# binbinmeng/QCNN_GPU

Hardware: NVIDIA B200
Metric: luma Mpixel/s (QVRCNN int8, 1080p) (higher is better)
Workload: dtype int8

## Files before the change

### include/qvrcnn_b200.h

```cpp
#ifndef QVRCNN_B200_H
#define QVRCNN_B200_H

#include <stddef.h>
#include <stdint.h>

#ifdef __cplusplus
extern "C" {
#endif

#if defined(__GNUC__)
#define QV_API __attribute__((visibility("default")))
#else
#define QV_API
#endif

typedef struct qv_net qv_net;

enum {
    QV_OK = 0,
    QV_ERR_ARG = -1,
    QV_ERR_IO = -2,
    QV_ERR_CUDA = -3,
    QV_ERR_RANGE = -4,
    QV_ERR_STATE = -5
// ... 15 lines not shown
QV_API int qv_destroy(qv_net *net);

QV_API int qv_load_static_para(qv_net *net, const char *filename);
QV_API int qv_load_static_para_mem(qv_net *net, const void *image, size_t len);
QV_API int qv_load_static_para_hwcn(qv_net *net, const char *filename);

QV_API int qv_load_quant_params(qv_net *net, const char *filename);
QV_API int qv_read_quant_params(const char *filename, int32_t *out18);
QV_API int qv_set_weights(qv_net *net, int layer, const int8_t *w_kcrs, const int32_t *bias);
QV_API int qv_get_quant_params(const qv_net *net, int32_t *out18);

QV_API int qv_load_data(qv_net *net, const uint8_t *host_luma);
QV_API int qv_forward_blu(qv_net *net);
QV_API int qv_get_recon(qv_net *net, uint8_t *host_out);

QV_API int qv_forward_frames_host(qv_net *net, const uint8_t *h_in, uint8_t *h_out, int n_frames);
QV_API int qv_stream_yuv(qv_net *net, const char *anchor_yuv, const char *ori_yuv, const char *recon_yuv,
                         int first_frame, int n_frames, int64_t *sse_before, int64_t *sse_after);
QV_API int qv_stream_yuv_pf(qv_net *net, const char *anchor_yuv, const char *ori_yuv, const char *recon_yuv,
                            int first_frame, int n_frames, int64_t *sse_before_pf, int64_t *sse_after_pf);
QV_API int qv_forward_frames_device(qv_net *net, const uint8_t *d_in, uint8_t *d_out, int n_frames,
                                    void *cuda_stream);
QV_API int qv_forward_frames_device_sse(qv_net *net, const uint8_t *d_in, const uint8_t *d_ori, uint8_t *d_out,
                                        int n_frames, int64_t *d_sse, void *cuda_stream);
QV_API int qv_forward_rows_device(qv_net *net, const uint8_t *d_in, int img_height, int in_row0, int in_rows,
                                  uint8_t *d_out, int out_row0, int out_row1, void *cuda_stream);

QV_API int qv_synchronize(qv_net *net, void *cuda_stream);

typedef struct { unsigned char opaque[192]; } qv_strip_desc;
enum { QV_STRIP_ABOVE = 0, QV_STRIP_BELOW = 1 };
QV_API int qv_strip_setup(qv_net *net, int img_height, int row0, int row1);
QV_API int qv_strip_export(qv_net *net, qv_strip_desc *out);
QV_API int qv_strip_attach(qv_net *net, int side, const qv_strip_desc *neighbour);
QV_API int qv_strip_input(qv_net *net, int slot, void **d_rows);
QV_API int qv_strip_acquire(qv_net *net, int slot, void *cuda_stream);
QV_API int qv_strip_load(qv_net *net, int slot, const uint8_t *host_rows, void *cuda_stream);
QV_API int qv_strip_forward(qv_net *net, int slot, uint8_t *d_out, void *cuda_stream);
QV_API int qv_strip_forward_sse(qv_net *net, int slot, const uint8_t *d_ori_rows, uint8_t *d_out, int64_t *d_sse2,
                                void *cuda_stream);
QV_API int qv_strip_release(qv_net *net);

QV_API int qv_device_buffers(qv_net *net, void **d_x, void **d_x_rec);

QV_API int qv_sse_device(const uint8_t *d_a, const uint8_t *d_b, size_t n, int64_t *d_sse_accum, void *cuda_stream);

QV_API int qv_set_impl(qv_net *net, int impl);
QV_API int qv_get_impl(const qv_net *net);
QV_API long long qv_launch_count(const qv_net *net);
QV_API int qv_get_activation(qv_net *net, int which , int8_t *host_out);

QV_API int qv_debug_fused_tables(const void *model_image, size_t len, uint8_t *wimg, uint32_t *ops, int32_t *consts, size_t sizes[3]);

QV_API int qv_debug_fused_units(int sm_count, int n_frames, int height, int width, int row0, int row1, int row_window, int allow_line,
                                int32_t *units, size_t *n_units, int *grid);

QV_API int qv_convert_model_hwcn_to_vect_c(const char *file_in, const char *file_out);

QV_API int qv_solve_quant_params(const double *stepw_in, const double *blu_in, double *rows_out36);
QV_API int qv_write_quant_params_cpp(const char *filename, const double *rows36);
QV_API int qv_quantize_layer(const float *w, size_t n_w, const float *b, size_t n_b, double stepw, double ratio,
                             int8_t *w_q, int32_t *b_q);

QV_API void *qv_host_alloc(size_t bytes);
QV_API void qv_host_free(void *p);

QV_API int qv_yuv_read_luma(const char *filename, int frames, int height, int width, uint8_t *out);
QV_API int qv_yuv_read_frame(const char *filename, int n, int height, int width, uint8_t *out);
QV_API int qv_yuv_write_recon(const char *filename, const uint8_t *luma, int frames, int height, int width);
QV_API double qv_psnr(const uint8_t *data, const uint8_t *ori, size_t n, int64_t *sse_out);
QV_API double qv_psnr_from_sse(int64_t sse, size_t n);

#ifdef __cplusplus
}
#endif
#endif
```

### qcnn_gpu_b200/api.py

```python
from __future__ import annotations

import ctypes as C
import os
from typing import Optional

import numpy as np

_PKG = os.path.dirname(os.path.abspath(__file__))
LIB_PATH = os.environ.get("QVRCNN_B200_LIB", os.path.join(_PKG, "libqvrcnn_b200.so"))

IMPL_AUTO, IMPL_LAYERED, IMPL_FUSED = 0, 1, 2

ABI_SYMBOLS = (
    "qv_last_error", "qv_version", "qv_create", "qv_destroy", "qv_load_static_para",
    "qv_load_static_para_mem", "qv_load_static_para_hwcn", "qv_load_quant_params", "qv_read_quant_params",
    "qv_set_weights", "qv_get_quant_params", "qv_load_data", "qv_forward_blu", "qv_get_recon",
    "qv_forward_frames_host", "qv_stream_yuv", "qv_stream_yuv_pf", "qv_forward_frames_device", "qv_forward_frames_device_sse", "qv_forward_rows_device", "qv_device_buffers",
    "qv_sse_device", "qv_host_alloc", "qv_host_free",
    "qv_set_impl", "qv_get_impl", "qv_launch_count", "qv_get_activation",
    "qv_convert_model_hwcn_to_vect_c", "qv_yuv_read_luma", "qv_yuv_read_frame", "qv_yuv_write_recon",
    "qv_psnr", "qv_psnr_from_sse", "qv_solve_quant_params", "qv_write_quant_params_cpp", "qv_quantize_layer",
    "qv_debug_fused_tables", "qv_debug_fused_units", "qv_synchronize",
    "qv_strip_setup", "qv_strip_export", "qv_strip_attach", "qv_strip_input", "qv_strip_acquire", "qv_strip_load",
    "qv_strip_forward", "qv_strip_forward_sse", "qv_strip_release",
)

CUDA_STREAM_LEGACY = 1
STRIP_ABOVE, STRIP_BELOW = 0, 1
STRIP_DESC_BYTES = 192


def stream_arg(stream: int):
    return CUDA_STREAM_LEGACY if not stream else stream


class QVError(RuntimeError):
    def __init__(self, code: int, msg: str):
        super().__init__("qvrcnn_b200 error %d: %s" % (code, msg))
        self.code = code


_lib = None


def lib():
    global _lib
    if _lib is None:
        if not os.path.exists(LIB_PATH):
            raise ImportError("%s not found: build it with `python -c 'import __graft_entry__ as g; g.build()'` "
                              "(there is no fallback implementation)" % LIB_PATH)
        L = C.CDLL(LIB_PATH)
        vp, i32, cp = C.c_void_p, C.c_int, C.c_char_p
        L.qv_last_error.restype = cp
        L.qv_version.restype = cp
        L.qv_create.argtypes = [i32, i32, i32, i32, i32, C.POINTER(vp)]
        L.qv_destroy.argtypes = [vp]
        L.qv_load_static_para.argtypes = [vp, cp]
        L.qv_load_static_para_mem.argtypes = [vp, vp, C.c_size_t]
        L.qv_load_static_para_hwcn.argtypes = [vp, cp]
        L.qv_load_quant_params.argtypes = [vp, cp]
        L.qv_read_quant_params.argtypes = [cp, vp]
        L.qv_set_weights.argtypes = [vp, i32, vp, vp]
        L.qv_get_quant_params.argtypes = [vp, vp]
        L.qv_load_data.argtypes = [vp, vp]
        L.qv_forward_blu.argtypes = [vp]
        L.qv_get_recon.argtypes = [vp, vp]
        L.qv_forward_frames_host.argtypes = [vp, vp, vp, i32]
        L.qv_forward_frames_device.argtypes = [vp, vp, vp, i32, vp]
        L.qv_forward_frames_device_sse.argtypes = [vp, vp, vp, vp, i32, vp, vp]
        L.qv_host_alloc.argtypes = [C.c_size_t]
        L.qv_host_alloc.restype = vp
        L.qv_host_free.argtypes = [vp]
        L.qv_host_free.restype = None
        L.qv_stream_yuv.argtypes = [vp, cp, cp, cp, i32, i32, C.POINTER(C.c_int64), C.POINTER(C.c_int64)]
        L.qv_stream_yuv_pf.argtypes = [vp, cp, cp, cp, i32, i32, vp, vp]
# ... 257 lines not shown
```

### qcnn_gpu_b200/csrc/qv_api.cu

```cuda
#include <algorithm>
#include <atomic>
#include <condition_variable>
#include <cstdio>
#include <cstdlib>
#include <cstring>
#include <mutex>
#include <random>
#include <thread>
#include <vector>

#include <fcntl.h>
#include <unistd.h>

#include <cuda_runtime.h>

#include "qv_fused.h"
#include "qv_internal.h"
#include "qv_layered.h"

using namespace qv;

#define QV_CUDA(expr)                                                                       \
    do {                                                                                    \
        cudaError_t e__ = (expr);                                                           \
// ... 243 lines not shown
    *out = net;
    return QV_OK;
}

int qv_destroy(qv_net *net)
{
    if (!net) return QV_OK;
    cudaSetDevice(net->dev);
    if (net->st) cudaStreamSynchronize(net->st);
    qv_strip_release(net);
    free_layered(net);
    if (net->fm) fused_free(net->fm);
    cudaFree(net->d_x); cudaFree(net->d_rec);
    cudaFree(net->d_a1); cudaFree(net->d_a2); cudaFree(net->d_a3);
    cudaFree(net->d_rows_tmp);
    for (int i = 0; i < 2; ++i) {
        cudaFree(net->d_slot_in[i]); cudaFree(net->d_slot_out[i]);
        cudaFreeHost(net->h_pin_in[i]); cudaFreeHost(net->h_pin_out[i]);
        if (net->pst[i]) cudaStreamDestroy(net->pst[i]);
    }
    if (net->ev_compute) cudaEventDestroy(net->ev_compute);
    if (net->st) cudaStreamDestroy(net->st);
    delete net;
    return QV_OK;
}

int qv_load_static_para_mem(qv_net *net, const void *image, size_t len)
{
    if (!net || !image) { set_error("qv_load_static_para_mem: null argument"); return QV_ERR_ARG; }
    ModelHost m;
    int rc = parse_model_vect_c((const uint8_t *)image, len, m);
    if (rc) return rc;
    net->model = m;
    return sync_model(net);
}

int qv_debug_fused_tables(const void *image, size_t len, uint8_t *wimg, uint32_t *ops, int32_t *consts, size_t sizes[3])
{
    if (!image || !sizes) { set_error("qv_debug_fused_tables: null argument"); return QV_ERR_ARG; }
    ModelHost m;
    int rc = parse_model_vect_c((const uint8_t *)image, len, m);
    if (rc) return rc;
    std::vector<uint8_t> w;
    std::vector<uint32_t> o;
    std::vector<int32_t> c;
    fused_debug_tables(m, w, o, c);
    if (wimg && sizes[0] >= w.size()) memcpy(wimg, w.data(), w.size());
    if (ops && sizes[1] >= o.size()) memcpy(ops, o.data(), o.size() * sizeof(uint32_t));
    if (consts && sizes[2] >= c.size()) memcpy(consts, c.data(), c.size() * sizeof(int32_t));
    sizes[0] = w.size(); sizes[1] = o.size(); sizes[2] = c.size();
    return QV_OK;
}

int qv_debug_fused_units(int sm_count, int n_frames, int height, int width, int row0, int row1, int row_window, int allow_line,
                         int32_t *units, size_t *n_units, int *grid)
{
    if (!n_units || !grid) { set_error("qv_debug_fused_units: null argument"); return QV_ERR_ARG; }
    std::vector<int> u;
    int g = 0;
    if (fused_debug_units(sm_count, n_frames, height, width, row0, row1, row_window != 0, allow_line != 0, u, g)) {
        set_error("qv_debug_fused_units: bad geometry");
        return QV_ERR_ARG;
    }
    if (units && *n_units >= u.size() / 5) memcpy(units, u.data(), u.size() * sizeof(int));
    *n_units = u.size() / 5;
    *grid = g;
    return QV_OK;
}

int qv_load_static_para(qv_net *net, const char *filename)
{
    if (!net) { set_error("qv_load_static_para: null handle"); return QV_ERR_ARG; }
    std::vector<uint8_t> buf;
    int rc = read_file(filename, buf);
    if (rc) { set_error("cannot open model file. (%s)", filename ? filename : "(null)"); return rc; }
    return qv_load_static_para_mem(net, buf.data(), buf.size());
}

int qv_load_static_para_hwcn(qv_net *net, const char *filename)
{
    if (!net) { set_error("qv_load_static_para_hwcn: null handle"); return QV_ERR_ARG; }
    std::vector<uint8_t> buf;
    int rc = read_file(filename, buf);
    if (rc) return rc;
    ModelHost m;
    rc = parse_model_hwcn(buf.data(), buf.size(), m);
    if (rc) return rc;
    net->model = m;
    return sync_model(net);
}

int qv_load_quant_params(qv_net *net, const char *filename)
{
    if (!net) { set_error("qv_load_quant_params: null handle"); return QV_ERR_ARG; }
    int32_t q[18];
    int rc = qv_read_quant_params(filename, q);
    if (rc) return rc;
    for (int l = 0; l < QV_NLAYER; ++l) {
        LayerHost &L = net->model.L[l];
        L.blu = q[3 * l]; L.mul = q[3 * l + 1]; L.shift = q[3 * l + 2];
        L.have_q = true;
    }
    return sync_model(net);
}

int qv_set_weights(qv_net *net, int layer, const int8_t *w_kcrs, const int32_t *bias)
// ... 719 lines not shown
```

### qcnn_gpu_b200/csrc/qv_fused.cu

```cuda
#include <algorithm>
#include <cstdio>
#include <cstdlib>
#include <cstring>
#include <mutex>
#include <type_traits>
#include <vector>

#include <cuda.h>
#include <cuda_runtime.h>

#include "qv_device.cuh"
#include "qv_fused.h"
#include "qv_tcgen05.cuh"


#ifndef QV_EXP
#define QV_EXP 0
#endif
#ifndef QV_CODE_SHIFT
#define QV_CODE_SHIFT 5
#endif
#ifndef QV_SHIFT_WORK
#define QV_SHIFT_WORK 0
#endif
#ifndef QV_SHIFT_C4
#define QV_SHIFT_C4 0
#endif
#ifndef QV_BULK_WEIGHTS
#define QV_BULK_WEIGHTS 1
#endif
#ifndef QV_LIGHT_PROF
#define QV_LIGHT_PROF 0
#endif

namespace qv {
namespace {
using namespace tc;
constexpr int EXP = QV_EXP;

constexpr int WT = 120;
constexpr int PW = 136;
constexpr int PLANE = PW * 16;
constexpr int A_SLOTS = 3, IN_SLOTS = 32, IN_PITCH = 144;
constexpr int A1_ROW = 4 * PLANE, A2_ROW = 3 * PLANE;
constexpr int IM_BYTES = 2 * 128 * 16;
constexpr int ZERO_BYTES = 2 * 128 * 16;

constexpr int NR22 = 11 * 16, NR21 = 7 * 32, NR31 = 7 * 16, NR32 = 32;
constexpr int W1_BYTES = 2 * 64 * 16;
constexpr int T22 = 2 * NR22 * 16, T21 = 2 * NR21 * 16, T31 = 2 * NR31 * 16, T32 = 2 * NR32 * 16;
constexpr int OFF_W1 = 0;
constexpr int OFF_W22 = OFF_W1 + W1_BYTES;
constexpr int OFF_W21 = OFF_W22 + 10 * T22;
constexpr int OFF_W31 = OFF_W21 + 6 * T21;
constexpr int OFF_W32 = OFF_W31 + 5 * T31;
constexpr int OFF_BIAS = OFF_W32 + 2 * T32;
constexpr int BIAS_INTS = 64 + 48 + 48;
constexpr int WIMG_BYTES = OFF_BIAS + BIAS_INTS * 4;
constexpr int OFF_A1 = (WIMG_BYTES + 127) / 128 * 128;
constexpr int OFF_A2 = OFF_A1 + A_SLOTS * A1_ROW;
constexpr int OFF_IM = OFF_A2 + A_SLOTS * A2_ROW;
constexpr int OFF_ZERO = OFF_IM + 3 * IM_BYTES;
constexpr int OFF_IN = OFF_ZERO + ZERO_BYTES;
constexpr int OFF_A3 = (OFF_IN + IN_SLOTS * IN_PITCH + 15) / 16 * 16;
constexpr int OFF_CTRL = OFF_A3 + A_SLOTS * A2_ROW;
constexpr int SMEM_BYTES = OFF_CTRL + 64;
static_assert(SMEM_BYTES <= 232448, "exceeds the 227 KB of dynamic shared memory per CTA");
constexpr int IN_PITCH_T = 256, IN_BOX = 144;
constexpr int OFF_IN_T = (SMEM_BYTES + 127) / 128 * 128;
constexpr int SMEM_BYTES_T = OFF_IN_T + IN_SLOTS * IN_PITCH_T;
static_assert(SMEM_BYTES_T <= 232448, "exceeds the 227 KB of dynamic shared memory per CTA");

#ifndef QV_ONE_WORKER
#define QV_ONE_WORKER 1
#endif
constexpr int NWORKER = QV_ONE_WORKER ? 128 : 256, NC4 = 128, NTHREADS = NWORKER + 32 + NC4;
constexpr int MMA_WARP = NWORKER / 32;
constexpr int TR_ITER0 = 300, TR_N = 8;
constexpr int PIPE = 14;

constexpr int TM_D1 = 0;
constexpr int TM_R22 = 128;
constexpr int TM_R21 = 224;
constexpr int TM_R31 = 352;
constexpr int TM_D32 = 416;
constexpr int TM_COLS = 512;

struct GroupQ {
    int hi;
    unsigned M;
    int blu, mul, shift, rbias;
};

struct alignas(64) FusedParams {
    CUtensorMap tmap_in;
    const uint8_t *in;
    uint8_t *out;
    const uint8_t *wimg;
    int n_frames, H, W, nstrips, nseg, seg_rows, n_units, linear, perm_q, perm_s0, perm_r;
    int ys, ye, own0, own1, rlo, rhi;
    size_t frame_stride;
    const uint8_t *in_top, *in_bot;
    const uint32_t *flag_top, *flag_bot;
    uint32_t *pub, *done, *done_ctr;
    uint32_t seq;
    GroupQ q1, q22, q21, q31, q32;
    int c4_bias, c4_mul, c4_shift;
    int c4_w[108];
    long long *dbg;
    uint32_t sbase16, tmem_base;
    int *fail_flag;
    int dbg_flags;
    int bias[BIAS_INTS];
    const uint8_t *ori;
    unsigned long long *sse;
};

struct PhaseBases {
    uint32_t im, a1_r2, a2_r6, b22;
    uint32_t b21, b31, d1, d32;
    uint32_t z22, z21, z31, pad;
};
struct FixedBases { uint32_t zeroA, w1, w32, r22, r21, r31, pad0, pad1; };
constexpr int N_PHASE = 12;
constexpr int N_MMA = 27;
struct PhaseOps {
    uint4 ab[N_MMA];
    uint32_t d1, d32, z22, z21, z31, pad[3];
};
__constant__ PhaseOps c_ops[N_PHASE];

__host__ __device__ __forceinline__ int mod_pos(int a, int m) { int r = a % m; return r < 0 ? r + m : r; }

__host__ __device__ __forceinline__ int wrap_sub(int c, int k, int n) { const int v = c - (k % n); return v < 0 ? v + n : v; }
__host__ __device__ __forceinline__ int wrap_inc(int c, int n) { return c + 1 == n ? 0 : c + 1; }

__device__ __forceinline__ void warp_wait(uint64_t *bar, uint32_t parity, int lane, int *fail)
{
    if (lane == 0 && !tc::mbar_wait(bar, parity)) *fail = 1;
    __syncwarp();
}

__device__ __forceinline__ bool peer_wait(const uint32_t *flag, uint32_t seq)
{
    for (int n = 0; n < 4000000; ++n) {
        uint32_t v;
        asm volatile("ld.acquire.sys.global.u32 %0, [%1];" : "=r"(v) : "l"(flag) : "memory");
        if ((int)(v - seq) >= 0) return true;
        __nanosleep(200);
    }
    return false;
}

struct UnitGeo { int strip, f, y0, y1; bool ok; };
template <bool ROWS>
__host__ __device__ __forceinline__ UnitGeo unit_geo(const FusedParams &P, int unit, int H, int grid)
{
    UnitGeo g;
    if (!ROWS && P.linear) {
        const int b = unit % grid, j = unit / grid;
        const int lo = b * P.seg_rows, hi = min(P.n_frames * P.nstrips * H, lo + P.seg_rows), c = lo / H + j;
        const int start = j == 0 ? lo : c * H, end = min(hi, (c + 1) * H);
        const int full = P.perm_r * (P.perm_s0 + 1);
        const int q = c < full ? c / (P.perm_s0 + 1) : P.perm_r + (c - full) / P.perm_s0;
        const int sl = c < full ? c - q * (P.perm_s0 + 1) : (c - full) - (q - P.perm_r) * P.perm_s0;
        const int col = q + sl * P.perm_q;
        g.f = col / P.nstrips;
        g.strip = col - g.f * P.nstrips;
        g.y0 = start - c * H;
        g.y1 = g.y0 + (end - start);
        g.ok = start < end;
    } else if (!ROWS) {
        const int seg = unit % P.nseg;
        g.strip = (unit / P.nseg) % P.nstrips;
        g.f = unit / (P.nseg * P.nstrips);
        g.y0 = seg * P.seg_rows;
        g.y1 = min(H, g.y0 + P.seg_rows);
        g.ok = true;
    } else {
        const int R = P.ye - P.ys, b = unit % grid, j = unit / grid;
        const int lo = b * P.seg_rows, hi = min(P.nstrips * R, lo + P.seg_rows), c0 = lo / R;
        const int start = j == 0 ? lo : (c0 + j) * R, end = min(hi, (c0 + j + 1) * R);
        g.strip = c0 + j;
// ... 48 lines not shown
    for (int dy = 0; dy < 3; ++dy)
#pragma unroll
        for (int pl = 0; pl < 3; ++pl) {
            const int *w = &P.c4_w[((dy * 3 + DX) * 3 + pl) * 4];
            acc[dy] = __dp4a((int)v[pl].x, w[0], acc[dy]);
            acc[dy] = __dp4a((int)v[pl].y, w[1], acc[dy]);
            acc[dy] = __dp4a((int)v[pl].z, w[2], acc[dy]);
            acc[dy] = __dp4a((int)v[pl].w, w[3], acc[dy]);
        }
}

template <bool FAST, bool PROF, bool ROWS, bool TMA = false>
__global__ void __launch_bounds__(NTHREADS, 1) k_fused(const __grid_constant__ FusedParams P)
{
    constexpr bool SSE = false;
#include "qv_fused_body.inc"
}

template <bool FAST, bool ROWS>
__global__ void __launch_bounds__(NTHREADS, 1) k_enh_sse(const __grid_constant__ FusedParams P)
{
    constexpr bool SSE = true, PROF = false, TMA = false;
#include "qv_fused_body.inc"
}

__global__ void k_wait_words(const uint32_t *a, uint32_t va, const uint32_t *b, uint32_t vb, int *fail_flag)
{
    const uint32_t *w = threadIdx.x == 0 ? a : b;
    const uint32_t v = threadIdx.x == 0 ? va : vb;
    if (w && !peer_wait(w, v)) { *reinterpret_cast<volatile int *>(fail_flag) = 3; __threadfence_system(); }
}

__global__ void k_bases(uint32_t *out)
{
    extern __shared__ __align__(1024) uint8_t sm[];
    uint32_t *slot = reinterpret_cast<uint32_t *>(sm);
    tmem_alloc(slot, TM_COLS);
    tmem_relinquish();
    fence_before_sync();
    __syncwarp();
    fence_after_sync();
    const uint32_t tm = *slot;
    if (threadIdx.x == 0) { out[0] = smem_u32(sm); out[1] = tm; }
    __syncwarp();
    tmem_dealloc(tm, TM_COLS);
}

void build_mma_bases(uint32_t sb, uint32_t tm, PhaseBases *pb, FixedBases &fb)
{
    constexpr uint32_t LP = (uint32_t)(PLANE >> 4) << 16;
    const uint32_t w22 = sb + (OFF_W22 >> 4) + ((uint32_t)NR22 << 16), w21 = sb + (OFF_W21 >> 4) + ((uint32_t)NR21 << 16);
    const uint32_t w31 = sb + (OFF_W31 >> 4) + ((uint32_t)NR31 << 16);
    fb = FixedBases{};
    fb.zeroA = sb + (OFF_ZERO >> 4) + ((128u * 16 >> 4) << 16);
    fb.w1 = sb + (OFF_W1 >> 4) + (64u << 16);
    fb.w32 = sb + (OFF_W32 >> 4) + ((uint32_t)NR32 << 16);
    fb.r22 = tm + TM_R22; fb.r21 = tm + TM_R21; fb.r31 = tm + TM_R31;
    for (int ph = 0; ph < N_PHASE; ++ph) {
        const int R1p = ph + 4096 / N_PHASE * N_PHASE + N_PHASE, c3 = ph % 3, c6 = ph % 6;
        const uint32_t par = ph & 1;
        const int qa = wrap_sub(c6, 2, 6);
        PhaseBases &e = pb[ph];
        e = PhaseBases{};
        e.im = sb + ((OFF_IM + c3 * IM_BYTES) >> 4) + ((128u * 16 >> 4) << 16);
        e.a1_r2 = sb + (OFF_A1 >> 4) + wrap_sub(c3, 2, 3) * (A1_ROW >> 4) + LP;
        e.a2_r6 = sb + (OFF_A2 >> 4) + c3 * (A2_ROW >> 4);
        e.b22 = w22 + (qa <= 2 ? 2 - qa : 8 - qa) * 16;
        e.b21 = w21 + ((1 - (R1p - 2)) & 3) * 32;
        e.b31 = w31 + ((1 - (R1p - 6)) & 3) * 16;
        e.d1 = tm + TM_D1 + par * 64; e.d32 = tm + TM_D32 + par * 32;
        e.z22 = tm + TM_R22 + c6 * 16;
        e.z21 = tm + TM_R21 + ((R1p - 1) & 3) * 32;
        e.z31 = tm + TM_R31 + ((R1p - 5) & 3) * 16;
    }
}

void build_mma_ops(const PhaseBases *pb, const FixedBases &fb, PhaseOps *ops)
{
    constexpr uint32_t HI = (128u >> 4) | (1u << 14);
    constexpr uint32_t LP = (uint32_t)(PLANE >> 4) << 16, LX = 1u << 16;
    for (int ph = 0; ph < N_PHASE; ++ph) {
        const PhaseBases &e = pb[ph];
        PhaseOps &o = ops[ph];
        o = PhaseOps{};
        int k = 0;
        auto put = [&](uint32_t a, uint32_t b) { o.ab[k++] = make_uint4(a, HI, b, HI); };
        put(e.im, fb.w1);
        put(fb.zeroA, fb.w1); put(fb.zeroA, fb.w1); put(fb.zeroA, fb.w1);
        put(e.a2_r6 + 6 + LP, e.b31);
        put(e.a2_r6 + 7 + LP, e.b31 + (T31 >> 4));
        put(e.a2_r6 + 7 + LP, fb.w32);
        put(e.a2_r6 + 8 + LP, e.b31 + 2 * (T31 >> 4));
        put(e.a2_r6 + ((2 * PLANE) >> 4) + 6 + LX, e.b31 + 3 * (T31 >> 4));
        put(e.a2_r6 + ((2 * PLANE) >> 4) + 6 + LX, fb.w32 + (T32 >> 4));
        put(e.a2_r6 + ((2 * PLANE) >> 4) + 8 + LX, e.b31 + 4 * (T31 >> 4));
        for (int t = 0; t < 10; ++t) {
            const int sft = t / 2, h = t & 1;
            const uint32_t a = e.a1_r2 + ((h * 2 * PLANE + (4 + sft) * 16) >> 4);
            put(a, e.b22 + t * (T22 >> 4));
            if (sft >= 1 && sft <= 3) put(a, e.b21 + ((sft - 1) * 2 + h) * (T21 >> 4));
        }
        o.d1 = e.d1; o.d32 = e.d32; o.z22 = e.z22; o.z21 = e.z21; o.z31 = e.z31;
    }
}

}

struct FusedModel {
    int *h_fail = nullptr;
    uint8_t *d_wimg = nullptr;
    FusedParams proto{};
    bool fast = true;
    int sm_count = 148;
    bool env_profile = false, env_test_fail = false, env_tma = false, env_linear = true;
    int env_experiment = 0;
    void *encode_tiled = nullptr;
};

static std::mutex g_ops_mu;
struct OpsRecord { bool done = false; uint32_t sbase16 = 0, tmem_base = 0; };
static OpsRecord g_ops_done[64];

static void put_chunk(uint8_t *blk, int NR, int j, int n, const int8_t *src16) { memcpy(blk + ((size_t)j * NR + n) * 16, src16, 16); }

static bool build_host_image(const ModelHost &m, std::vector<uint8_t> &img, FusedParams &P)
{
    img.assign(WIMG_BYTES, 0);
    auto Wt = [&](int l, int k, int c, int r, int s) -> int8_t {
        const LayerShape &sh = kLayers[l];
        return m.L[l].w[(((size_t)k * sh.cin + c) * sh.k + r) * sh.k + s];
    };
    for (int n = 0; n < 64; ++n) {
        int8_t k32[32] = {0};
        for (int r = 0; r < 5; ++r) {
            for (int s = 0; s < 4; ++s) k32[4 * r + s] = Wt(QV_C1, n, 0, r, s);
            k32[20 + r] = Wt(QV_C1, n, 0, r, 4);
        }
        put_chunk(img.data() + OFF_W1, 64, 0, n, k32);
        put_chunk(img.data() + OFF_W1, 64, 1, n, k32 + 16);
    }
    const int S22[11] = {4, 3, 2, 1, 0, -1, 4, 3, 2, 1, 0};
    const int S3[7] = {2, 1, 0, -1, 2, 1, 0};
    int8_t c16[16];
    for (int s = 0; s < 5; ++s)
        for (int h = 0; h < 2; ++h) {
            uint8_t *blk = img.data() + OFF_W22 + (s * 2 + h) * T22;
            for (int bi = 0; bi < 11; ++bi)
                if (S22[bi] >= 0)
                    for (int j = 0; j < 2; ++j)
                        for (int ch = 0; ch < 16; ++ch) {
                            for (int b = 0; b < 16; ++b) c16[b] = Wt(QV_C2_2, ch, 32 * h + 16 * j + b, S22[bi], s);
                            put_chunk(blk, NR22, j, bi * 16 + ch, c16);
                        }
        }
// ... 27 lines not shown
                }
    for (int ch = 0; ch < 32; ++ch)
        for (int pl = 0; pl < 3; ++pl) {
            for (int b = 0; b < 16; ++b) c16[b] = Wt(QV_C3_2, ch, 16 * pl + b, 0, 0);
            put_chunk(img.data() + OFF_W32 + (pl / 2) * T32, NR32, pl == 2 ? 1 : pl, ch, c16);
        }
    auto mkq = [&](int l, GroupQ &g) -> bool {
        const LayerHost &L = m.L[l];
        g.blu = L.blu; g.mul = L.mul; g.shift = L.shift; g.rbias = (1 << (L.shift - 1)) / L.mul;
        g.hi = L.blu + g.rbias;
        const long long top = ((long long)L.blu + g.rbias) * L.mul;
        const bool ok = L.shift <= 24 && L.mul < (1ll << L.shift) && top < (1ll << 31) && (top >> L.shift) == 127 && g.hi < (1 << 30);
        g.M = ok ? (unsigned)((unsigned long long)L.mul << (24 - L.shift)) : 0u;
        return ok;
    };
    bool fast = true;
    fast &= mkq(QV_C1, P.q1); fast &= mkq(QV_C2_2, P.q22); fast &= mkq(QV_C2_1, P.q21);
    fast &= mkq(QV_C3_1, P.q31); fast &= mkq(QV_C3_2, P.q32);
    int *bias = reinterpret_cast<int *>(img.data() + OFF_BIAS);
    auto addb = [&](int l, int dst0, const GroupQ &g) {
        for (int k = 0; k < kLayers[l].cout; ++k) bias[dst0 + k] = m.L[l].b[k] + (fast ? g.rbias : 0);
    };
    addb(QV_C1, 0, P.q1);
    addb(QV_C2_2, 64, P.q22); addb(QV_C2_1, 64 + 16, P.q21);
    addb(QV_C3_1, 112, P.q31); addb(QV_C3_2, 112 + 16, P.q32);
    memcpy(P.bias, bias, sizeof(P.bias));
    P.c4_bias = m.L[QV_C4].b[0]; P.c4_mul = m.L[QV_C4].mul; P.c4_shift = m.L[QV_C4].shift;
    for (int t = 0; t < 9; ++t)
        for (int pl = 0; pl < 3; ++pl)
            for (int j = 0; j < 4; ++j) {
                unsigned v = 0;
                for (int b = 0; b < 4; ++b) v |= (unsigned)(uint8_t)Wt(QV_C4, 0, 16 * pl + 4 * j + b, t / 3, t % 3) << (8 * b);
                P.c4_w[(t * 3 + pl) * 4 + j] = (int)v;
            }
    return fast;
}

void fused_debug_tables(const ModelHost &m, std::vector<uint8_t> &wimg, std::vector<uint32_t> &ops, std::vector<int32_t> &consts)
{
    FusedParams P{};
    const bool fast = build_host_image(m, wimg, P);
    PhaseBases pb[N_PHASE];
    FixedBases fb;
    build_mma_bases(0, 0, pb, fb);
    std::vector<PhaseOps> po(N_PHASE);
    build_mma_ops(pb, fb, po.data());
    ops.assign(reinterpret_cast<const uint32_t *>(po.data()), reinterpret_cast<const uint32_t *>(po.data() + N_PHASE));
    consts = {WIMG_BYTES, SMEM_BYTES, OFF_A1, OFF_A2, OFF_IM, OFF_ZERO, OFF_IN, OFF_A3, PW, PLANE, A1_ROW, A2_ROW, IM_BYTES, IN_SLOTS,
              IN_PITCH, WT, PIPE, TM_D1, TM_R22, TM_R21, TM_R31, TM_D32, N_PHASE, N_MMA, fast ? 1 : 0, P.c4_bias, P.c4_mul, P.c4_shift};
    for (const GroupQ *g : {&P.q1, &P.q22, &P.q21, &P.q31, &P.q32})
        for (int v : {g->hi, (int)g->M, g->blu, g->mul, g->shift, g->rbias}) consts.push_back(v);
    consts.insert(consts.end(), P.bias, P.bias + BIAS_INTS);
    consts.insert(consts.end(), P.c4_w, P.c4_w + 108);
}

FusedModel *fused_upload(const ModelHost &m, cudaStream_t st)
{
    std::vector<uint8_t> img;
    FusedModel *fm = new FusedModel();
    FusedParams &P = fm->proto;
    fm->fast = build_host_image(m, img, P);
    cudaError_t e = cudaMalloc(&fm->d_wimg, WIMG_BYTES);
    if (e == cudaSuccess) e = cudaMemcpyAsync(fm->d_wimg, img.data(), WIMG_BYTES, cudaMemcpyHostToDevice, st);
    if (e == cudaSuccess) e = cudaStreamSynchronize(st);
    if (e == cudaSuccess) e = cudaFuncSetAttribute(k_fused<true, false, false>, cudaFuncAttributeMaxDynamicSharedMemorySize, SMEM_BYTES);
    if (e == cudaSuccess) e = cudaFuncSetAttribute(k_fused<false, false, false>, cudaFuncAttributeMaxDynamicSharedMemorySize, SMEM_BYTES);
    if (e == cudaSuccess) e = cudaFuncSetAttribute(k_fused<true, false, true>, cudaFuncAttributeMaxDynamicSharedMemorySize, SMEM_BYTES);
    if (e == cudaSuccess) e = cudaFuncSetAttribute(k_fused<false, false, true>, cudaFuncAttributeMaxDynamicSharedMemorySize, SMEM_BYTES);
    if (e == cudaSuccess) e = cudaFuncSetAttribute(k_fused<true, true, false>, cudaFuncAttributeMaxDynamicSharedMemorySize, SMEM_BYTES);
    if (e == cudaSuccess) e = cudaFuncSetAttribute(k_fused<true, false, false, true>, cudaFuncAttributeMaxDynamicSharedMemorySize, SMEM_BYTES_T);
    if (e == cudaSuccess) e = cudaFuncSetAttribute(k_enh_sse<true, false>, cudaFuncAttributeMaxDynamicSharedMemorySize, SMEM_BYTES);
    if (e == cudaSuccess) e = cudaFuncSetAttribute(k_enh_sse<false, false>, cudaFuncAttributeMaxDynamicSharedMemorySize, SMEM_BYTES);
    if (e == cudaSuccess) e = cudaFuncSetAttribute(k_enh_sse<true, true>, cudaFuncAttributeMaxDynamicSharedMemorySize, SMEM_BYTES);
    if (e == cudaSuccess) e = cudaFuncSetAttribute(k_enh_sse<false, true>, cudaFuncAttributeMaxDynamicSharedMemorySize, SMEM_BYTES);
    if (e == cudaSuccess) e = cudaFuncSetAttribute(k_bases, cudaFuncAttributeMaxDynamicSharedMemorySize, SMEM_BYTES);
    int dev = 0, sms = 148;
    if (e == cudaSuccess) e = cudaGetDevice(&dev);
    if (e == cudaSuccess && (dev < 0 || dev >= 64)) e = cudaErrorInvalidDevice;
    if (e == cudaSuccess) {
        std::lock_guard<std::mutex> lock(g_ops_mu);
        OpsRecord &rec = g_ops_done[dev];
        if (!rec.done) {
            uint32_t *d_b = nullptr, h_b[2] = {0, 0};
            e = cudaMalloc(&d_b, 8);
            if (e == cudaSuccess) {
                k_bases<<<1, 32, SMEM_BYTES, st>>>(d_b);
                e = cudaMemcpyAsync(h_b, d_b, 8, cudaMemcpyDeviceToHost, st);
                if (e == cudaSuccess) e = cudaStreamSynchronize(st);
                cudaFree(d_b);
            }
            if (e == cudaSuccess) {
                PhaseBases pb[N_PHASE];
                FixedBases fb;
                build_mma_bases(h_b[0] >> 4, h_b[1], pb, fb);
                std::vector<PhaseOps> ops(N_PHASE);
                build_mma_ops(pb, fb, ops.data());
                e = cudaMemcpyToSymbolAsync(c_ops, ops.data(), sizeof(PhaseOps) * N_PHASE, 0, cudaMemcpyHostToDevice, st);
                if (e == cudaSuccess) e = cudaStreamSynchronize(st);
                if (e == cudaSuccess) { rec.done = true; rec.sbase16 = h_b[0] >> 4; rec.tmem_base = h_b[1]; }
            }
        }
        P.sbase16 = rec.sbase16; P.tmem_base = rec.tmem_base;
    }
    if (e == cudaSuccess) e = cudaDeviceGetAttribute(&sms, cudaDevAttrMultiProcessorCount, dev);
    if (e != cudaSuccess) {
        set_error("fused_upload: %s", cudaGetErrorString(e));
// ... 227 lines not shown
```

### qcnn_gpu_b200/csrc/qv_fused.h

```cpp
#pragma once
#include <cstdint>
#include <vector>
#include <cuda_runtime.h>

#include "qv_internal.h"

namespace qv {

struct FusedModel;

FusedModel *fused_upload(const ModelHost &m, cudaStream_t st);
void fused_free(FusedModel *fm);
struct FusedRows {
    int own0 = 0, own1 = 0, out0 = 0, out1 = 0, top_rows = 0, bot_rows = 0;
    const uint8_t *d_top = nullptr, *d_bot = nullptr;
    const uint32_t *flag_top = nullptr, *flag_bot = nullptr;
    uint32_t *pub = nullptr, *done = nullptr, *done_ctr = nullptr;
    uint32_t seq = 0;
};
constexpr int FUSED_SSE_MAX_H = 66051;
cudaError_t fused_forward(const FusedModel *fm, const uint8_t *d_in, uint8_t *d_out, int n, int H, int W,
                          cudaStream_t st, long long *launches, const FusedRows *rows = nullptr,
                          const uint8_t *d_ori = nullptr, int64_t *d_sse = nullptr);
cudaError_t fused_wait_words(const FusedModel *fm, const uint32_t *a, uint32_t va, const uint32_t *b, uint32_t vb, cudaStream_t st);
int fused_take_failure(const FusedModel *fm);

void fused_debug_tables(const ModelHost &m, std::vector<uint8_t> &wimg, std::vector<uint32_t> &ops, std::vector<int32_t> &consts);
int fused_debug_units(int sm_count, int n_frames, int H, int W, int row0, int row1, bool rows_mode, bool allow_linear, std::vector<int> &units, int &grid);

}
```

### qcnn_gpu_b200/csrc/qv_fused_body.inc

```
    static_assert(!(TMA && ROWS), "the TMA input ring exists for whole-frame launches only");
    static_assert(!(SSE && (TMA || PROF)), "no SSE form of the TMA input ring or of the profiling build");
    constexpr int IN_BASE = TMA ? OFF_IN_T : OFF_IN, IN_ROWPITCH = TMA ? IN_PITCH_T : IN_PITCH;
    extern __shared__ __align__(1024) uint8_t sm[];
    uint64_t *bar_mma = reinterpret_cast<uint64_t *>(sm + OFF_CTRL);
    uint32_t *s_tmem = reinterpret_cast<uint32_t *>(sm + OFF_CTRL + 32);
    int *s_fail = reinterpret_cast<int *>(sm + OFF_CTRL + 36);
    const int tid = threadIdx.x, warp = tid >> 5, lane = tid & 31;
    const int H = P.H, W = P.W;

    if (ROWS && P.pub && blockIdx.x == 0 && tid == 0) asm volatile("st.release.sys.global.u32 [%0], %1;" ::"l"(P.pub), "r"(P.seq) : "memory");
#pragma unroll
    for (int j = 0; j < QV_CODE_SHIFT; ++j) asm volatile("membar.cta;" ::: "memory");
#if QV_BULK_WEIGHTS
    static_assert(WIMG_BYTES % 16 == 0 && WIMG_BYTES < (1 << 20), "cp.async.bulk size / mbarrier tx-count");
    uint64_t *bar_in = reinterpret_cast<uint64_t *>(sm + OFF_CTRL + 40);
    uint64_t *bar_w = reinterpret_cast<uint64_t *>(sm + OFF_CTRL + 56);
    if (tid == 0) {
        mbar_init(&bar_mma[0], 1);
        mbar_init(&bar_mma[1], 1);
        if (TMA) { mbar_init(&bar_in[0], 1); mbar_init(&bar_in[1], 1); }
        mbar_init(bar_w, 1);
        *s_fail = 0;
        mbar_fence_init();
        constexpr uint32_t PART = (WIMG_BYTES / 4 + 15) / 16 * 16;
        asm volatile("mbarrier.arrive.expect_tx.shared::cta.b64 _, [%0], %1;" ::"r"(smem_u32(bar_w)), "r"((uint32_t)WIMG_BYTES) : "memory");
#pragma unroll
        for (uint32_t o = 0; o < (uint32_t)WIMG_BYTES; o += PART) {
            const uint32_t n = o + PART <= (uint32_t)WIMG_BYTES ? PART : (uint32_t)WIMG_BYTES - o;
            asm volatile("cp.async.bulk.shared::cluster.global.mbarrier::complete_tx::bytes [%0], [%1], %2, [%3];"
                         ::"r"(smem_u32(sm + o)), "l"(P.wimg + o), "r"(n), "r"(smem_u32(bar_w)) : "memory");
        }
    }
    for (int i = tid; i < (OFF_CTRL - OFF_A1) / 16; i += NTHREADS)
        reinterpret_cast<uint4 *>(sm + OFF_A1)[i] = make_uint4(0, 0, 0, 0);
    if (tid == 0 && !tc::mbar_wait(bar_w, 0)) *s_fail = 1;
#else
    for (int i = tid; i < WIMG_BYTES / 16; i += NTHREADS)
        reinterpret_cast<uint4 *>(sm)[i] = reinterpret_cast<const uint4 *>(P.wimg)[i];
    for (int i = tid; i < (OFF_CTRL - OFF_A1) / 16; i += NTHREADS)
        reinterpret_cast<uint4 *>(sm + OFF_A1)[i] = make_uint4(0, 0, 0, 0);
    uint64_t *bar_in = reinterpret_cast<uint64_t *>(sm + OFF_CTRL + 40);
    if (tid == 0) {
        mbar_init(&bar_mma[0], 1);
        mbar_init(&bar_mma[1], 1);
        if (TMA) { mbar_init(&bar_in[0], 1); mbar_init(&bar_in[1], 1); }
        *s_fail = 0;
        mbar_fence_init();
    }
#endif
    if (warp == MMA_WARP) { tmem_alloc(s_tmem, TM_COLS); tmem_relinquish(); }
    fence_proxy_async_smem();
    fence_before_sync();
    __syncthreads();
    fence_after_sync();
    const uint32_t tm = *s_tmem;
    const uint32_t sbase = smem_u32(sm);

    if (warp == MMA_WARP) {
        const bool leader = elect_one();
        uint32_t nb3 = 0, ev_mma = 0;
        long long t_wait = 0, t_issue = 0, tc0 = PROF ? clock64() : 0;
        const bool issue = leader && !(PROF && (P.dbg_flags & 1));
        long long *stamp = nullptr;
        constexpr std::integral_constant<int, COL_DISCARD> ONCE{};
        constexpr std::integral_constant<int, COL_FILL> KEEP{};
        constexpr std::integral_constant<int, COL_USE> AGAIN{};
        constexpr std::integral_constant<int, COL_LASTUSE> LAST{};
        if ((sbase >> 4) != P.sbase16 || tm != P.tmem_base) { if (lane == 0) *s_fail = 2; }
        const uint32_t r22 = tm + TM_R22, r21 = tm + TM_R21, r31 = tm + TM_R31;
        for (int unit = blockIdx.x; unit < P.n_units; unit += gridDim.x) {
            const UnitGeo g = unit_geo<ROWS>(P, unit, H, (int)gridDim.x);
            if (!g.ok) continue;
            const int y0 = g.y0, y1 = g.y1;
            const int niter = y1 - y0 + PIPE;
            int ph = mod_pos(y0 - 4, N_PHASE);
            for (int i = 0; i < niter; ++i) {
                const PhaseOps &op = c_ops[ph];
                auto MMA = [&](auto col, uint32_t d, int k, uint32_t idesc, uint32_t acc) {
                    const uint4 ab = op.ab[k];
                    if (issue) mma_i8_ss_col<decltype(col)::value>(d, ((uint64_t)ab.y << 32) | ab.x, ((uint64_t)ab.w << 32) | ab.z, idesc, acc);
                    if (PROF && stamp) *stamp++ = clock64();
                };
                asm volatile("bar.sync %0, %1;" ::"r"(2u + nb3), "n"(NWORKER + NC4 + 32) : "memory");
                nb3 = nb3 == 2 ? 0 : nb3 + 1;
                fence_after_sync();
                bool tr = false;
                if (PROF) {
                    const long long t = clock64(); t_wait += t - tc0; tc0 = t;
                    tr = P.dbg && leader && unit == 0 && i >= TR_ITER0 && i < TR_ITER0 + TR_N;
                    if (tr) P.dbg[gridDim.x * 16 + (i - TR_ITER0) * 16 + 0] = tc0;
                    stamp = (tr && !QV_LIGHT_PROF) ? P.dbg + gridDim.x * 16 + TR_N * 16 + (i - TR_ITER0) * 32 : nullptr;
                }
                MMA(ONCE, op.d1, 0, idesc_i8(128, 64), 0);
                MMA(KEEP, op.z22, 1, idesc_i8(128, 16), 0);
                MMA(AGAIN, op.z21, 2, idesc_i8(128, 32), 0);
                MMA(LAST, op.z31, 3, idesc_i8(128, 16), 0);
                MMA(ONCE, r31, 4, idesc_i8(128, 64), 1);
                MMA(KEEP, r31, 5, idesc_i8(128, 64), 1);
                MMA(LAST, op.d32, 6, idesc_i8(128, 32), 0);
                MMA(ONCE, r31, 7, idesc_i8(128, 64), 1);
                MMA(KEEP, r31, 8, idesc_i8(128, 64), 1);
                MMA(LAST, op.d32, 9, idesc_i8(128, 32), 1);
                MMA(ONCE, r31, 10, idesc_i8(128, 64), 1);
                int k = 11;
#pragma unroll
                for (int t = 0; t < 10; ++t) {
                    const int s = t / 2;
                    if (s >= 1 && s <= 3) {
                        MMA(KEEP, r22, k++, idesc_i8(128, 96), 1);
                        MMA(LAST, r21, k++, idesc_i8(128, 128), 1);
                    } else {
                        MMA(ONCE, r22, k++, idesc_i8(128, 96), 1);
                    }
                }
                ph = wrap_inc(ph, N_PHASE);
                if (leader) mma_commit(&bar_mma[ev_mma & 1]);
                ++ev_mma;
                __syncwarp();
                if (PROF) {
                    const long long t = clock64(); t_issue += t - tc0; tc0 = t;
                    if (tr) P.dbg[gridDim.x * 16 + (i - TR_ITER0) * 16 + 1] = tc0;
                }
            }
        }
        if (PROF && P.dbg && leader) { P.dbg[blockIdx.x * 16 + 0] = t_wait; P.dbg[blockIdx.x * 16 + 1] = t_issue; }
    } else if (warp < NWORKER / 32) {
#pragma unroll
        for (int j = 0; j < QV_SHIFT_WORK; ++j) asm volatile("membar.cta;" ::: "memory");
        const int q = warp & 3, hh = warp >> 2;
        const int m = q * 32 + lane;
        const uint32_t tm_lane = tm + ((uint32_t)(q * 32) << 16);
        uint32_t ev_work = 0, ev_mma = 0;
        long long tw[6] = {0, 0, 0, 0, 0, 0}, tc0 = PROF ? clock64() : 0, t_ldtm = 0;
        int tr_slot = -1;
        auto lap = [&](int k) {
            if (PROF && QV_LIGHT_PROF) {
                if (tr_slot >= 0 && k < 4) P.dbg[gridDim.x * 16 + tr_slot + k] = clock64();
            } else if (PROF) {
                const long long t = clock64(); tw[k] += t - tc0; tc0 = t;
                if (tr_slot >= 0 && k < 4) P.dbg[gridDim.x * 16 + tr_slot + k] = t;
            }
        };
        auto worker_bar = []() { asm volatile("bar.sync 1, %0;" ::"n"(NWORKER + NC4) : "memory"); };
        for (int unit = blockIdx.x; unit < P.n_units; unit += gridDim.x) {
            const UnitGeo g = unit_geo<ROWS>(P, unit, H, (int)gridDim.x);
            if (!g.ok) continue;
            const int strip = g.strip, f = g.f, y0 = g.y0, y1 = g.y1;
            const int X0 = strip * WT;
            const int niter = y1 - y0 + PIPE;
            worker_bar();
            work_arrive(ev_work);
            ++ev_work;
            int c3 = mod_pos(y0 - 4, 3), c6 = mod_pos(y0 - 4, 6);
            const bool xa1 = (unsigned)(X0 - 4 + m) < (unsigned)W, xa2 = (unsigned)(X0 - 2 + m) < (unsigned)W, xa3 = (unsigned)(X0 - 1 + m) < (unsigned)W;
            for (int i = 0; i < niter; ++i, c3 = wrap_inc(c3, 3), c6 = wrap_inc(c6, 6)) {
                const int R1 = y0 - 4 + i, R1p = R1 + 4096;
                if (PROF)
                    tr_slot = (P.dbg && unit == 0 && (tid == 0 || tid == NWORKER / 2) && i >= TR_ITER0 && i < TR_ITER0 + TR_N)
                                  ? (i - TR_ITER0) * 16 + 2 + (tid / (NWORKER / 2)) * 4 : -1;
                if (PROF && i >= 1 && (P.dbg_flags & 2)) {
                    warp_wait(&bar_mma[ev_mma & 1], (ev_mma >> 1) & 1, lane, s_fail);
                    ++ev_mma;
                    fence_after_sync();
                    lap(0);
                } else if (i >= 1) {
                    warp_wait(&bar_mma[ev_mma & 1], (ev_mma >> 1) & 1, lane, s_fail);
                    ++ev_mma;
// ... 268 lines not shown
```

Before: 21740.

## Reorder tcgen05 MMA issue so zero-init slots reuse collector A operands

Replaces the hand-written MMA issue sequence with a table-driven order (kFusedIssueOrder) checked at compile time. The three zero-initialisation MMAs now use the A operand of the next MMA plus a zero B tile, so the collector buffer can be filled and reused by the following accumulating MMA. This replaces the separate zero-A loads. It also changes QV_CODE_SHIFT from 5 to 2 and adds a debug API that exports the issue order. The reordering changes when the ring accumulators are first written, which is guarded by static asserts.

```diff
diff --git a/include/qvrcnn_b200.h b/include/qvrcnn_b200.h
--- a/include/qvrcnn_b200.h
+++ b/include/qvrcnn_b200.h
@@ -91,6 +91,8 @@
 
 QV_API int qv_debug_fused_tables(const void *model_image, size_t len, uint8_t *wimg, uint32_t *ops, int32_t *consts, size_t sizes[3]);
 
+QV_API int qv_debug_fused_issue_order(int32_t *order, size_t *n);
+
 QV_API int qv_debug_fused_units(int sm_count, int n_frames, int height, int width, int row0, int row1, int row_window, int allow_line,
                                 int32_t *units, size_t *n_units, int *grid);
 
diff --git a/qcnn_gpu_b200/api.py b/qcnn_gpu_b200/api.py
--- a/qcnn_gpu_b200/api.py
+++ b/qcnn_gpu_b200/api.py
@@ -20,7 +20,7 @@
     "qv_set_impl", "qv_get_impl", "qv_launch_count", "qv_get_activation",
     "qv_convert_model_hwcn_to_vect_c", "qv_yuv_read_luma", "qv_yuv_read_frame", "qv_yuv_write_recon",
     "qv_psnr", "qv_psnr_from_sse", "qv_solve_quant_params", "qv_write_quant_params_cpp", "qv_quantize_layer",
-    "qv_debug_fused_tables", "qv_debug_fused_units", "qv_synchronize",
+    "qv_debug_fused_tables", "qv_debug_fused_issue_order", "qv_debug_fused_units", "qv_synchronize",
     "qv_strip_setup", "qv_strip_export", "qv_strip_attach", "qv_strip_input", "qv_strip_acquire", "qv_strip_load",
     "qv_strip_forward", "qv_strip_forward_sse", "qv_strip_release",
 )
diff --git a/qcnn_gpu_b200/csrc/qv_api.cu b/qcnn_gpu_b200/csrc/qv_api.cu
--- a/qcnn_gpu_b200/csrc/qv_api.cu
+++ b/qcnn_gpu_b200/csrc/qv_api.cu
@@ -319,6 +319,16 @@
     return QV_OK;
 }
 
+int qv_debug_fused_issue_order(int32_t *order, size_t *n)
+{
+    if (!n) { set_error("qv_debug_fused_issue_order: null argument"); return QV_ERR_ARG; }
+    std::vector<int32_t> o;
+    fused_debug_issue_order(o);
+    if (order && *n >= o.size()) memcpy(order, o.data(), o.size() * sizeof(int32_t));
+    *n = o.size();
+    return QV_OK;
+}
+
 int qv_debug_fused_units(int sm_count, int n_frames, int height, int width, int row0, int row1, int row_window, int allow_line,
                          int32_t *units, size_t *n_units, int *grid)
 {
diff --git a/qcnn_gpu_b200/csrc/qv_fused.cu b/qcnn_gpu_b200/csrc/qv_fused.cu
--- a/qcnn_gpu_b200/csrc/qv_fused.cu
+++ b/qcnn_gpu_b200/csrc/qv_fused.cu
@@ -4,6 +4,7 @@
 #include <cstring>
 #include <mutex>
 #include <type_traits>
+#include <utility>
 #include <vector>
 
 #include <cuda.h>
@@ -18,7 +19,7 @@
 #define QV_EXP 0
 #endif
 #ifndef QV_CODE_SHIFT
-#define QV_CODE_SHIFT 5
+#define QV_CODE_SHIFT 2
 #endif
 #ifndef QV_SHIFT_WORK
 #define QV_SHIFT_WORK 0
@@ -121,14 +122,52 @@
     uint32_t b21, b31, d1, d32;
     uint32_t z22, z21, z31, pad;
 };
-struct FixedBases { uint32_t zeroA, w1, w32, r22, r21, r31, pad0, pad1; };
+struct FixedBases { uint32_t zero, w1, w32, r22, r21, r31, pad0, pad1; };
 constexpr int N_PHASE = 12;
-constexpr int N_MMA = 27;
+constexpr int N_MMA = FUSED_N_MMA;
 struct PhaseOps {
     uint4 ab[N_MMA];
     uint32_t d1, d32, z22, z21, z31, pad[3];
 };
 __constant__ PhaseOps c_ops[N_PHASE];
+
+enum SlotAcc : uint8_t { ACC_D1, ACC_Z22, ACC_Z21, ACC_Z31, ACC_D32, ACC_R31, ACC_R22, ACC_R21 };
+struct SlotShape { uint8_t acc_at, n, accumulate; };
+constexpr SlotShape kSlotShape[N_MMA] = {
+    {ACC_D1, 64, 0},
+    {ACC_Z22, 16, 0}, {ACC_Z21, 32, 0}, {ACC_Z31, 16, 0},
+    {ACC_R31, 64, 1}, {ACC_R31, 64, 1}, {ACC_D32, 32, 0}, {ACC_R31, 64, 1}, {ACC_R31, 64, 1}, {ACC_D32, 32, 1}, {ACC_R31, 64, 1},
+    {ACC_R22, 96, 1}, {ACC_R22, 96, 1},
+    {ACC_R22, 96, 1}, {ACC_R21, 128, 1}, {ACC_R22, 96, 1}, {ACC_R21, 128, 1},
+    {ACC_R22, 96, 1}, {ACC_R21, 128, 1}, {ACC_R22, 96, 1}, {ACC_R21, 128, 1},
+    {ACC_R22, 96, 1}, {ACC_R21, 128, 1}, {ACC_R22, 96, 1}, {ACC_R21, 128, 1},
+    {ACC_R22, 96, 1}, {ACC_R22, 96, 1},
+};
+static_assert(COL_DISCARD == 0 && COL_FILL == 1 && COL_USE == 2 && COL_LASTUSE == 3, "kFusedIssueOrder's hint numbering");
+
+constexpr int issue_pos(int slot)
+{
+    for (int p = 0; p < N_MMA; ++p)
+        if (kFusedIssueOrder[p].slot == slot) return p;
+    return -1;
+}
+constexpr bool issue_order_ok()
+{
+    for (int s = 0; s < N_MMA; ++s)
+        if (issue_pos(s) < 0) return false;
+    for (int z = 1; z <= 3; ++z) {
+        const int p = issue_pos(z);
+        if (kFusedIssueOrder[p].col != COL_FILL || p + 1 >= N_MMA || kFusedIssueOrder[p + 1].col != COL_LASTUSE) return false;
+        const uint8_t ring = z == 1 ? ACC_R22 : z == 2 ? ACC_R21 : ACC_R31;
+        for (int q = 0; q < p; ++q)
+            if (kSlotShape[kFusedIssueOrder[q].slot].acc_at == ring) return false;
+    }
+    return true;
+}
+static_assert(issue_order_ok(), "kFusedIssueOrder");
+
+template <class F, int... I>
+__device__ __forceinline__ void for_each_index(F &&f, std::integer_sequence<int, I...>) { (f(std::integral_constant<int, I>{}), ...); }
 
 __host__ __device__ __forceinline__ int mod_pos(int a, int m) { int r = a % m; return r < 0 ? r + m : r; }
 
@@ -283,7 +322,7 @@
     const uint32_t w22 = sb + (OFF_W22 >> 4) + ((uint32_t)NR22 << 16), w21 = sb + (OFF_W21 >> 4) + ((uint32_t)NR21 << 16);
     const uint32_t w31 = sb + (OFF_W31 >> 4) + ((uint32_t)NR31 << 16);
     fb = FixedBases{};
-    fb.zeroA = sb + (OFF_ZERO >> 4) + ((128u * 16 >> 4) << 16);
+    fb.zero = sb + (OFF_ZERO >> 4) + ((128u * 16 >> 4) << 16);
     fb.w1 = sb + (OFF_W1 >> 4) + (64u << 16);
     fb.w32 = sb + (OFF_W32 >> 4) + ((uint32_t)NR32 << 16);
     fb.r22 = tm + TM_R22; fb.r21 = tm + TM_R21; fb.r31 = tm + TM_R31;
@@ -317,7 +356,7 @@
         int k = 0;
         auto put = [&](uint32_t a, uint32_t b) { o.ab[k++] = make_uint4(a, HI, b, HI); };
         put(e.im, fb.w1);
-        put(fb.zeroA, fb.w1); put(fb.zeroA, fb.w1); put(fb.zeroA, fb.w1);
+        k = 4;
         put(e.a2_r6 + 6 + LP, e.b31);
         put(e.a2_r6 + 7 + LP, e.b31 + (T31 >> 4));
         put(e.a2_r6 + 7 + LP, fb.w32);
@@ -331,6 +370,7 @@
             put(a, e.b22 + t * (T22 >> 4));
             if (sft >= 1 && sft <= 3) put(a, e.b21 + ((sft - 1) * 2 + h) * (T21 >> 4));
         }
+        for (int z = 1; z <= 3; ++z) o.ab[z] = make_uint4(o.ab[kFusedIssueOrder[issue_pos(z) + 1].slot].x, HI, fb.zero, HI);
         o.d1 = e.d1; o.d32 = e.d32; o.z22 = e.z22; o.z21 = e.z21; o.z31 = e.z31;
     }
 }
@@ -464,6 +504,12 @@
         for (int v : {g->hi, (int)g->M, g->blu, g->mul, g->shift, g->rbias}) consts.push_back(v);
     consts.insert(consts.end(), P.bias, P.bias + BIAS_INTS);
     consts.insert(consts.end(), P.c4_w, P.c4_w + 108);
+}
+
+void fused_debug_issue_order(std::vector<int32_t> &order)
+{
+    order.clear();
+    for (const FusedIssue &s : kFusedIssueOrder) { order.push_back(s.slot); order.push_back(s.col); }
 }
 
 FusedModel *fused_upload(const ModelHost &m, cudaStream_t st)
diff --git a/qcnn_gpu_b200/csrc/qv_fused.h b/qcnn_gpu_b200/csrc/qv_fused.h
--- a/qcnn_gpu_b200/csrc/qv_fused.h
+++ b/qcnn_gpu_b200/csrc/qv_fused.h
@@ -25,7 +25,19 @@
 cudaError_t fused_wait_words(const FusedModel *fm, const uint32_t *a, uint32_t va, const uint32_t *b, uint32_t vb, cudaStream_t st);
 int fused_take_failure(const FusedModel *fm);
 
+struct FusedIssue { uint8_t slot, col; };
+constexpr int FUSED_N_MMA = 27;
+constexpr FusedIssue kFusedIssueOrder[FUSED_N_MMA] = {
+    {0, 0},
+    {3, 1}, {4, 3},
+    {5, 1}, {6, 3}, {7, 0}, {8, 1}, {9, 3}, {10, 0},
+    {1, 1}, {11, 3},
+    {2, 1}, {12, 3},
+    {13, 1}, {14, 3}, {15, 1}, {16, 3}, {17, 1}, {18, 3}, {19, 1}, {20, 3}, {21, 1}, {22, 3}, {23, 1}, {24, 3},
+    {25, 0}, {26, 0},
+};
 void fused_debug_tables(const ModelHost &m, std::vector<uint8_t> &wimg, std::vector<uint32_t> &ops, std::vector<int32_t> &consts);
+void fused_debug_issue_order(std::vector<int32_t> &order);
 int fused_debug_units(int sm_count, int n_frames, int H, int W, int row0, int row1, bool rows_mode, bool allow_linear, std::vector<int> &units, int &grid);
 
 }
diff --git a/qcnn_gpu_b200/csrc/qv_fused_body.inc b/qcnn_gpu_b200/csrc/qv_fused_body.inc
--- a/qcnn_gpu_b200/csrc/qv_fused_body.inc
+++ b/qcnn_gpu_b200/csrc/qv_fused_body.inc
@@ -62,10 +62,6 @@
         long long t_wait = 0, t_issue = 0, tc0 = PROF ? clock64() : 0;
         const bool issue = leader && !(PROF && (P.dbg_flags & 1));
         long long *stamp = nullptr;
-        constexpr std::integral_constant<int, COL_DISCARD> ONCE{};
-        constexpr std::integral_constant<int, COL_FILL> KEEP{};
-        constexpr std::integral_constant<int, COL_USE> AGAIN{};
-        constexpr std::integral_constant<int, COL_LASTUSE> LAST{};
         if ((sbase >> 4) != P.sbase16 || tm != P.tmem_base) { if (lane == 0) *s_fail = 2; }
         const uint32_t r22 = tm + TM_R22, r21 = tm + TM_R21, r31 = tm + TM_R31;
         for (int unit = blockIdx.x; unit < P.n_units; unit += gridDim.x) {
@@ -91,28 +87,15 @@
                     if (tr) P.dbg[gridDim.x * 16 + (i - TR_ITER0) * 16 + 0] = tc0;
                     stamp = (tr && !QV_LIGHT_PROF) ? P.dbg + gridDim.x * 16 + TR_N * 16 + (i - TR_ITER0) * 32 : nullptr;
                 }
-                MMA(ONCE, op.d1, 0, idesc_i8(128, 64), 0);
-                MMA(KEEP, op.z22, 1, idesc_i8(128, 16), 0);
-                MMA(AGAIN, op.z21, 2, idesc_i8(128, 32), 0);
-                MMA(LAST, op.z31, 3, idesc_i8(128, 16), 0);
-                MMA(ONCE, r31, 4, idesc_i8(128, 64), 1);
-                MMA(KEEP, r31, 5, idesc_i8(128, 64), 1);
-                MMA(LAST, op.d32, 6, idesc_i8(128, 32), 0);
-                MMA(ONCE, r31, 7, idesc_i8(128, 64), 1);
-                MMA(KEEP, r31, 8, idesc_i8(128, 64), 1);
-                MMA(LAST, op.d32, 9, idesc_i8(128, 32), 1);
-                MMA(ONCE, r31, 10, idesc_i8(128, 64), 1);
-                int k = 11;
-#pragma unroll
-                for (int t = 0; t < 10; ++t) {
-                    const int s = t / 2;
-                    if (s >= 1 && s <= 3) {
-                        MMA(KEEP, r22, k++, idesc_i8(128, 96), 1);
-                        MMA(LAST, r21, k++, idesc_i8(128, 128), 1);
-                    } else {
-                        MMA(ONCE, r22, k++, idesc_i8(128, 96), 1);
-                    }
-                }
+                auto issue_at = [&](auto pos) {
+                    constexpr FusedIssue s = kFusedIssueOrder[decltype(pos)::value];
+                    constexpr SlotShape sh = kSlotShape[s.slot];
+                    const uint32_t d = sh.acc_at == ACC_D1 ? op.d1 : sh.acc_at == ACC_Z22 ? op.z22 : sh.acc_at == ACC_Z21 ? op.z21
+                                     : sh.acc_at == ACC_Z31 ? op.z31 : sh.acc_at == ACC_D32 ? op.d32 : sh.acc_at == ACC_R31 ? r31
+                                     : sh.acc_at == ACC_R22 ? r22 : r21;
+                    MMA(std::integral_constant<int, s.col>{}, d, s.slot, idesc_i8(128, sh.n), sh.accumulate);
+                };
+                for_each_index(issue_at, std::make_integer_sequence<int, N_MMA>{});
                 ph = wrap_inc(ph, N_PHASE);
                 if (leader) mma_commit(&bar_mma[ev_mma & 1]);
                 ++ev_mma;
```

Measured after the change: 21690 (median of 6 runs). No clear change (-0.2%).
